# Potato256/my-mitsuba

Measured on AMD Instinct MI355X. Metric: Msamples/sec at 1280x720x256spp, 1/2/4/8 MI355X; per-pixel L1 vs CPU ref, higher is better.
Workload: dtype f32; 1 GPU; C3 bunny x15, 1,041,765 triangles, roughconductor Cu GGX 0.2, 15 instances flattened to world-space triangles; resolution=1280x720, spp=256, max_depth=8, parallelism=film tiles round-robin over 1 GPU(s), kd_build=host, kd_refs=4723933, kd_stop_prims=4

## Files before the change

include/mtsg.h:

```cpp
#ifndef MTSG_H
#define MTSG_H

#include <stdint.h>
#include <stddef.h>

#ifdef __cplusplus
extern "C" {
#endif

#define MTSG_ABI_VERSION 8

enum {
    MTSG_OK             = 0,
    MTSG_ERR_INVALID    = -1,
    MTSG_ERR_DEVICE     = -2,
    MTSG_ERR_OOM        = -3,
    MTSG_ERR_CANCELLED  = -4,
    MTSG_ERR_NODEVICE   = -5,
    MTSG_ERR_TRAVERSAL  = -6
};


typedef struct mtsg_kdnode {
    uint32_t combined;
// ... 333 lines not shown

int  mtsg_render_device(mtsg_scene *scene, const mtsg_render_params *params,
                        float *rgbaw_device);

int  mtsg_tile_windows(mtsg_scene *scene, const mtsg_render_params *params,
                       uint32_t *ntiles, int32_t *window);
int  mtsg_render_device_tiles(mtsg_scene *scene, const mtsg_render_params *params,
                              float *windows_device);

int  mtsg_set_tile_list(mtsg_scene *scene, const int32_t *keys, uint32_t n);

int  mtsg_device_alloc(mtsg_scene *scene, size_t bytes, void **out);
int  mtsg_device_free(mtsg_scene *scene, void *ptr);
int  mtsg_device_memset(mtsg_scene *scene, void *ptr, size_t bytes);
int  mtsg_device_to_host(mtsg_scene *scene, void *dst, const void *src, size_t bytes);

void mtsg_cancel(mtsg_scene *scene);

void mtsg_cancel_clear(mtsg_scene *scene);

typedef void (*mtsg_tile_fn)(void *user, int32_t key, int32_t x, int32_t y, int32_t w, int32_t h);
int  mtsg_set_tile_callback(mtsg_scene *scene, mtsg_tile_fn fn, void *user);

int  mtsg_set_flags(mtsg_scene *scene, uint32_t flags);
int  mtsg_get_stats(mtsg_scene *scene, mtsg_stats *out);
int  mtsg_debug_wavetimes(mtsg_scene *scene, uint64_t *out, uint32_t max_launches, uint32_t *waves);
int  mtsg_debug_stragglers(mtsg_scene *scene, float *out, uint32_t max_rays);

int  mtsg_set_batch_paths(mtsg_scene *scene, uint32_t paths);

#define MTSG_DEFAULT_FINISH_PATHS 524288u
int  mtsg_set_finish_paths(mtsg_scene *scene, uint32_t paths);

enum {
    MTSG_OPT_TRACE_REFILL = 1,
    MTSG_OPT_FINISH_SHADE_MIN = 2,
    MTSG_OPT_LANES = 3,
    MTSG_OPT_STAGGER = 4,
    MTSG_OPT_SHADE_GENERIC = 5,
    MTSG_OPT_RAY_ORDER = 6,
    MTSG_OPT_CAMERA_DIFFS = 7
};
int  mtsg_set_option(mtsg_scene *scene, int32_t key, int64_t value);

enum { MTSG_EMITTER_SET_AREA = 0, MTSG_EMITTER_SET_ENVMAP = 1, MTSG_EMITTER_SET_ALL = 2 };
int  mtsg_scene_kernel_sets(mtsg_scene *scene, int32_t *material_set, int32_t *emitter_set);

typedef struct mtsg_test_knobs {
    int32_t stack_cap, restart_guard, restart_limit, limit_shadow_only;
    int32_t no_instance_prefilter;
} mtsg_test_knobs;
int  mtsg_set_test_knobs(mtsg_scene *scene, const mtsg_test_knobs *knobs);

int  mtsg_env_eval(mtsg_scene *scene, uint32_t n, const float *dirs, const float *rx, const float *ry, float *out);

int  mtsg_tex_eval(mtsg_scene *scene, int tex, uint32_t n, const float *uv, const float *duv, float *out);

int  mtsg_om_query(mtsg_scene *scene, uint32_t n, const float *dirs, const float *o1, const float *o2, int32_t *ids,
                   int32_t *vis);

typedef struct mtsg_kd_build_params {
    float traversal_cost;
    float query_cost;
    float empty_space_bonus;
    int32_t stop_prims;
    int32_t max_depth;
    int32_t pad;
} mtsg_kd_build_params;

typedef struct mtsg_kd_tree {
    mtsg_kdnode *nodes;
    uint32_t n_nodes;
    uint32_t *indices;
    uint32_t n_indices;
// ... 88 lines not shown
```

my-mitsuba_amd/csrc/kernels.h:

```cpp
#pragma once
#include <hip/hip_runtime.h>

#include <stdint.h>

#include "../../include/mtsg.h"
#include "device_math.h"
#include "envmap.h"
#include "sampler.h"

namespace mtsg {

struct DevCamera;
struct DevScene {
    const uint4 *__restrict__ blocks;
    uint2 root2;
    const float4 *__restrict__ triL;
    const float4 *__restrict__ vpos;
    const float4 *__restrict__ vnrm;
    const uint4 *__restrict__ tidx;
    const float4 *__restrict__ shrec;
    const mtsg_rect *__restrict__ rects;
    const float4 *__restrict__ rectM;
    const float4 *__restrict__ rectSh;
    const float4 *__restrict__ emitRect;
    const mtsg_shape *__restrict__ shapes;
    const mtsg_bsdf *__restrict__ bsdfs;
    const mtsg_emitter *__restrict__ emitters;
    const float *__restrict__ emitter_cdf;
    const float *__restrict__ emitter_tri_cdf;
    uint32_t n_emitters, n_tri, n_bsdfs;
    float bmin[3], bmax[3];
    int has_env;
    DevEnv env;
    const uint32_t *qmcPrimes, *qmcOff;
    const uint16_t *qmcPerm;
    const float4 *__restrict__ inst;
    const mtsg_texture *__restrict__ textures;
    const float *__restrict__ tex_texels;
    const float4 *__restrict__ ttex;
    int cam_diffs;
    int cam_env_diffs;
    const DevCamera *__restrict__ camDev;
    float camO[3], camNear, camFar;
    int camCompact;
    uint4 *__restrict__ instSave;
    const mtsg_om *__restrict__ om;
    const uint32_t *__restrict__ om_bits;
    uint32_t capFlat, capGrp, capTop, rstGuard, rstMax, rstMaxC;
    uint32_t instPrefilter;
    uint32_t instKeyStride;
};

struct DevCamera {
    float s2c[16];
    float c2w[12];
// ... 64 lines not shown
    hipStream_t stream;
    const DevScene *S;
    const DevIntegrator *I;
    const DevBatch *B;
    const DevPaths *P;
    int bounce, qin;
    uint32_t nIdentity;
    int hasAlpha;
    uint32_t shadeMin;
    bool env, ext, inst;
    int mats;
    bool emx = false;
};
template <int SMP> void launch_shade_smp(const ShadeLaunch &a);
template <int SMP> void launch_finish_smp(const ShadeLaunch &a);
#define MTSG_DECLARE_LAUNCHERS(SMP) \
    template <> void launch_shade_smp<SMP>(const ShadeLaunch &a); \
    template <> void launch_finish_smp<SMP>(const ShadeLaunch &a);
MTSG_DECLARE_LAUNCHERS(MTSG_SAMPLER_INDEPENDENT)
MTSG_DECLARE_LAUNCHERS(MTSG_SAMPLER_HALTON)
MTSG_DECLARE_LAUNCHERS(MTSG_SAMPLER_HAMMERSLEY)
MTSG_DECLARE_LAUNCHERS(MTSG_SAMPLER_LDSAMPLER)
MTSG_DECLARE_LAUNCHERS(MTSG_SAMPLER_SOBOL)
int finish_blocks_per_cu(bool mats);
struct FlatTraceLaunch {
    dim3 grid, tieGrid;
    hipStream_t stream;
    const DevScene *S;
    const DevPaths *P;
    int cIn, sIn;
    uint32_t n;
    unsigned long long *wt;
    bool count, knobs, refill32, tie;
};
void launch_trace_flat(const FlatTraceLaunch &a);
int trace_flat_blocks_per_cu();

struct DevAov {
    int m;
    int pathChild;
    int nf;
    int kind[MTSG_MAX_SUBINTEGRATORS];
    int child[MTSG_MAX_SUBINTEGRATORS];
    float undef[MTSG_MAX_SUBINTEGRATORS][3];
    float w2c[16];
    const mtsg_aov_bsdf *bsdfs;
    const mtsg_aov_shape *shapes;
    const uint32_t *elems;
    float *planes;
    size_t cap;
};
struct FieldsLaunch {
    hipStream_t stream;
    const DevScene *S;
    const DevCamera *C;
    const DevIntegrator *I;
    const DevBatch *B;
    const DevPaths *P;
    const DevAov *A;
    float *film;
    int blockW, blockH, win;
};
void launch_fields(const FieldsLaunch &a);
void launch_splat_multi(const FieldsLaunch &a);

struct DevDirect {
// ... 387 lines not shown
    __syncthreads();
#endif
#if MTSG_LDS_PAD
    if (threadIdx.x == 0) ((volatile uint32_t *)s_ldsPad)[(S.n_tri & 0xFFFFu) % (MTSG_LDS_PAD / 4)] = 0u;
#endif
}
DEV uint32_t lane_here() {
    uint32_t l;
    asm volatile("v_mbcnt_lo_u32_b32 %0, -1, 0\n\tv_mbcnt_hi_u32_b32 %0, -1, %0" : "=v"(l));
    return l;
}
DEV uint32_t rank_below(unsigned long long m) {
    return __builtin_amdgcn_mbcnt_hi((uint32_t)(m >> 32), __builtin_amdgcn_mbcnt_lo((uint32_t)m, 0u));
}
struct SpecStack {
    DEV static uint32_t at(uint32_t k) { return k * TRACE_BLOCK + lane_here(); }
    DEV void push(uint32_t k, uint2 node, float t) const {
        const uint32_t i = at(k);
        s_specNode[i] = node;
        s_specT[i] = t;
    }
    DEV uint2 node(uint32_t k) const { return s_specNode[at(k)]; }
    DEV float t(uint32_t k) const { return s_specT[at(k)]; }
};

DEV float4 miss_record() {
    float4 m;
    uint32_t inf = 0x7F800000u, z = 0u, ff = 0xFFFFFFFFu;
    asm volatile("" : "+v"(inf), "+v"(z), "+v"(ff));
    m.x = __uint_as_float(inf); m.y = __uint_as_float(z); m.z = __uint_as_float(z); m.w = __uint_as_float(ff);
    return m;
}

DEV bool spec_init(const DevScene &S, float3 o, float3 d, float rayMint, float rayMaxt, bool shadow, SpecRay &r) {
    r.o = o;
    r.d = d;
    r.inv = mk3(rcp_exact(d.x), rcp_exact(d.y), rcp_exact(d.z));
    const uint32_t dneg = (d.x <= 0.0f ? 1u : 0u) | (d.y <= 0.0f ? 2u : 0u) | (d.z <= 0.0f ? 4u : 0u);
    float nearT = -INFINITY, farT = INFINITY;
    bool ok = true;
#pragma unroll
    for (int i = 0; i < 3; ++i) {
        const float oi = comp(o, i), di = comp(d, i), ii = comp(r.inv, i);
        const bool par = di == 0.0f;
        const float t1 = (S.bmin[i] - oi) * ii, t2 = (S.bmax[i] - oi) * ii;
        nearT = par ? nearT : fmaxf(fminf(t1, t2), nearT);
        farT = par ? farT : fminf(fmaxf(t1, t2), farT);
        ok &= !par | ((oi >= S.bmin[i]) & (oi <= S.bmax[i]));
    }
    if (!ok || !(nearT <= farT)) return false;
    float m = fmaxf(fmaxf(fabsf(o.x), fabsf(o.y)), fabsf(o.z));
    if (!shadow) m = fmaxf(m, kEpsilon);
    const float rayMinT = rayMint == kEpsilon ? rayMint * m : rayMint;
    r.mint = fmaxf(nearT, rayMinT);
    r.best = fminf(farT, rayMaxt);
    if (!(r.best > r.mint)) return false;
    r.tmin = r.mint;
    r.tmax = r.best;
    r.cur = S.root2;
    r.rroot = S.root2;
    r.lfE = r.lfEnd = 0;
    r.lfTmax = -1.0f;
    r.bits = dneg << SB_DNEG | (shadow ? SB_SHADOW : 0u);
    r.mb = 0;
    r.bestKey = 0xFFFFFFFFu;
    return true;
}

DEV void spec_plan(const SpecRay &r, uint2 n, float &tsplit, bool &goLeft, bool &push) {
    const uint32_t axis = n.x & 3u;
    const float split = __uint_as_float(n.y);
    const bool a0 = axis == 0u, a1 = axis == 1u;
    const float ox = r.o.x, oy = r.o.y, oz = r.o.z, ix = r.inv.x, iy = r.inv.y, iz = r.inv.z;
    const float oa = a0 ? ox : (a1 ? oy : oz);
    const float ia = a0 ? ix : (a1 ? iy : iz);
    tsplit = (split - oa) * ia;
    if (tsplit != tsplit) tsplit = INFINITY;
    const bool belowFirst = (oa < split) | ((oa == split) & (bool)((r.bits >> (SB_DNEG + axis)) & 1u));
    const bool onlyFirst = (tsplit > r.tmax) | (tsplit <= 0.0f);
    const bool goSecond = !onlyFirst & (tsplit < r.tmin);
    push = !onlyFirst & !goSecond;
    goLeft = belowFirst != goSecond;
}

#ifndef MTSG_PUSHDOWN
#define MTSG_PUSHDOWN 0
#endif
DEV uint2 spec_take(SpecRay &r, const uint4 &pr, float tsplit, bool goLeft, bool push, SpecStack stk, uint32_t cap) {
    const uint2 c = goLeft ? make_uint2(pr.x, pr.y) : make_uint2(pr.z, pr.w);
#if MTSG_PUSHDOWN
    if (!push && !(r.bits & (SB_N | SB_DROPPED))) r.rroot = c;
#endif
    if (push) {
        const uint2 other = goLeft ? make_uint2(pr.z, pr.w) : make_uint2(pr.x, pr.y);
        const uint32_t b = r.bits, top = b & SB_TOP;
        stk.push(top, other, r.tmax);
        const bool full = (b & SB_N) == cap * SB_N1;
        r.bits = ((b & ~SB_TOP) | (top == cap - 1 ? 0u : top + 1u)) + (full ? SB_DROPPED - (b & SB_DROPPED) : SB_N1);
// ... 1 lines not shown
    }
    return c;
}

#ifndef MTSG_RECT_PEND
#define MTSG_RECT_PEND 0
#endif
#ifndef MTSG_RECT_PEND_I
#define MTSG_RECT_PEND_I 0
#endif
#ifndef MTSG_ENTER_BATCH
#define MTSG_ENTER_BATCH 8
#endif
#ifndef MTSG_POPSEL
#define MTSG_POPSEL 0
#endif
#ifndef MTSG_INST_MIN_IDLE
#define MTSG_INST_MIN_IDLE 16
#endif
#ifndef MTSG_EXIT_BATCH
#define MTSG_EXIT_BATCH 0
#endif
#ifndef MTSG_MAILBOX
#define MTSG_MAILBOX 1
#endif
#ifndef MTSG_TIE_INLINE
#define MTSG_TIE_INLINE 0
#endif
constexpr bool TIE_INLINE = MTSG_TIE_INLINE;
#ifndef MTSG_RETIRE_BATCH
#define MTSG_RETIRE_BATCH 1
#endif
constexpr bool RETIRE_BATCH = MTSG_RETIRE_BATCH;
__shared__ uint32_t s_mbPrev[TRACE_BLOCK];
DEV bool mailbox_tie(SpecRay &r, uint32_t mb, uint32_t sl, uint32_t id, const float4 *hitOut) {
    if (!(r.bits & SB_FOUND)) return true;
    const uint32_t bs = (mb >> 20) & 7u, ps = (mb >> 17) & 7u;
    const uint32_t bestId = ((const uint32_t *)hitOut)[3];
    if (id == bestId) {
        r.mb = (mb & ~(1u << bs)) | (0x100u << bs);
        return false;
    }
    if ((mb & 0x10000u) && id == s_mbPrev[lane_here()] && !(mb & (0x100u << ps))) {
        r.mb = mb;
        return false;
    }
    s_mbPrev[lane_here()] = bestId;
    r.mb = sl << 20 | bs << 17 | 0x10000u | ((mb & 0xFFu) | (1u << sl)) << 8;
    return true;
}
DEV bool mailbox_step(SpecRay &r, uint32_t key, bool isRect, uint32_t prim, bool h, float t, const float4 *hitOut) {
    const uint32_t mb = r.mb, tag = (key & 7u) << 20 | 0x101u << (key & 7u);
    r.mb = h ? (tag & 0x700000u) : ((tag & 0xFFFFu) | mb);
    if (h & (t == r.best)) h = mailbox_tie(r, mb, tag >> 20, isRect ? (0x80000000u | prim) : prim, hitOut);
    return h;
}

template <bool COUNT, bool MB = false>
DEV bool spec_iter(const DevScene &S, SpecRay &r, SpecStack stk, TraceCounts &cnt, float4 *hitOut, const TravLimits &L) {
    const uint2 n = r.cur;
    const bool inner = !(r.bits & SB_TRAVDONE) && !(n.x & 0x80000000u);
    const bool prim = r.lfE < r.lfEnd;
    const bool rootKind = inner && !(n.x & 4u);
    float tsplit;
    bool goLeft, push;
    spec_plan(r, n, tsplit, goLeft, push);
    const uint32_t base = inner ? (n.x >> 3) << ((~n.x >> 1) & 2u) : 0u;
    const uint32_t off = rootKind ? 2u - (uint32_t)goLeft : 0u;
    const uint32_t pi = prim ? r.lfE : 0u;
#if MTSG_LDS_TOP
    uint4 p0, pc;
    if (base < 20u) p0 = s_top[base]; else p0 = S.blocks[base];
    if (base + off < 20u) pc = s_top[base + off]; else pc = S.blocks[base + off];
#else
    const uint4 p0 = S.blocks[base], pc = S.blocks[base + off];
#endif
#if MTSG_RECT_PEND
    const bool rp = (r.bits & SB_RPEND) != 0;
    const float4 *rec = rp ? S.rectM + (size_t)(3u * r.rpend) : S.triL + (size_t)(3u * pi);
#else
    const float4 *rec = S.triL + (size_t)(3u * pi);
#endif
    const float4 f0 = rec[0], f1 = rec[1], f2 = rec[2];
    asm volatile("" ::"v"(p0.x), "v"(p0.y), "v"(p0.z), "v"(p0.w), "v"(pc.x), "v"(pc.y), "v"(pc.z), "v"(pc.w),
                 "v"(f0.x), "v"(f0.y), "v"(f0.z), "v"(f0.w),
                 "v"(f1.x), "v"(f1.y), "v"(f1.z), "v"(f1.w), "v"(f2.x), "v"(f2.y), "v"(f2.z), "v"(f2.w));
#if MTSG_RECT_PEND
    if (prim && !rp && __float_as_uint(f0.x) == MTSG_TRIACCEL_SHAPE) {
        r.rpend = __float_as_uint(f2.w);
        r.bits |= SB_RPEND;
    } else if (prim) {
        if (COUNT) { cnt.refs++; cnt.tests++; }
        float t, u, v;
        const bool isRect = rp;
        bool h;
        uint32_t key, pid;
        if (rp) {
            h = rect_test_rows(f0, f1, f2, r.o, r.d, r.mint, r.best, t, u, v);
            key = S.n_tri + r.rpend;
            pid = r.rpend;
            r.bits &= ~SB_RPEND;
        } else {
            h = tri_test(f0, f1, f2, r.o, r.d, r.mint, r.best, u, v, t);
            key = __float_as_uint(f2.z);
            pid = __float_as_uint(f2.w);
        }
#else
    if (prim) {
        if (COUNT) { cnt.refs++; cnt.tests++; }
        float t, u, v;
        bool h = tri_test(f0, f1, f2, r.o, r.d, r.mint, r.best, u, v, t);
        const bool isRect = __float_as_uint(f0.x) == MTSG_TRIACCEL_SHAPE;
        if (isRect) h = rect_test(S.rects[__float_as_uint(f2.w)], r.o, r.d, r.mint, r.best, t, u, v);
        const uint32_t key = __float_as_uint(f2.z), pid = __float_as_uint(f2.w);
#endif
#if MTSG_MAILBOX
        if (MB) h = mailbox_step(r, key, isRect, pid, h, t, hitOut);
        else r.bits |= (h & (t == r.best) & (key != r.bestKey)) ? SB_TIE : 0u;
        if (h) r.bestKey = key;
#endif
        if (h) {
            r.bits |= SB_FOUND;
            if (r.bits & SB_SHADOW) return true;
            r.best = t;
            stS(hitOut, make_float4(t, u, v, __uint_as_float(isRect ? (0x80000000u | pid) : pid)));
        }
        ++r.lfE;
    }
    if (inner) {
        if (COUNT) cnt.nodes++;
        const uint2 c = spec_take(r, p0, tsplit, goLeft, push, stk, L.capFlat);
        r.cur = c;
        if (rootKind && !(c.x & 0x80000000u)) {
            if (COUNT) cnt.nodes++;
            float ts2;
            bool gl2, push2;
            spec_plan(r, c, ts2, gl2, push2);
            r.cur = spec_take(r, pc, ts2, gl2, push2, stk, L.capFlat);
        }
    }
    const bool found = (r.bits & SB_FOUND) != 0;
    const bool leafDone = (r.lfTmax >= 0.0f) & (r.lfE >= r.lfEnd);
    if (leafDone & found & (r.best < r.lfTmax)) return true;
    r.lfTmax = leafDone ? -1.0f : r.lfTmax;
    const uint2 c = r.cur;
// ... 586 lines not shown
            if (__lane_id() == 63u) waveSum[tid >> 6] = incl;
        }
        __syncthreads();
        if (tid < (uint32_t)SORT_BINS) {
            uint32_t before = 0u;
            for (uint32_t w = 0; w < (tid >> 6); ++w) before += waveSum[w];
            hist[tid] = before + incl - v;
        }
        __syncthreads();
#pragma unroll
        for (int j = 0; j < PER; ++j) {
            const uint32_t pos = w0 + (uint32_t)j * SORT_BLOCK + tid;
            if (pos < n) P.orderBuf[w0 + hist[key[j]] + rank[j]] = pos;
        }
        __syncthreads();
    }
}

#ifndef MTSG_SHUFFLE
#define MTSG_SHUFFLE 0
#endif
DEV uint32_t shuffle_index(uint32_t x, uint32_t n) {
    if (n < 2) return x;
    const uint32_t m = 32u - __clz(n - 1u), mask = m >= 32 ? 0xFFFFFFFFu : (1u << m) - 1u;
    do {
        x = (x * 0x9E3779B1u + 0x7F4A7C15u) & mask;
        x ^= x >> ((m + 1) / 2);
        x = (x * 0x85EBCA6Bu) & mask;
        x ^= x >> ((m + 2) / 3);
    } while (x >= n);
    return x;
}

template <bool COUNT, int MIN_IDLE, bool INST, bool KNOBS>
DEV void trace_s_body(const DevScene &S, const DevPaths &P, int cIn, int sIn, uint32_t nIdentity, unsigned long long *wt) {
    const SpecStack stk{};
    const TravLimits L = trav_limits<KNOBS>(S);
    lds_top_init(S);
    const unsigned long long tStart = wt ? wall_clock64() : 0ull;
    const uint32_t nC = cIn == -1 ? nIdentity : (cIn >= 0 ? __atomic_load_n(&P.cnt[cnt_q(cIn)], __ATOMIC_RELAXED) : 0u);
    const uint32_t nS = sIn >= 0 ? __atomic_load_n(&P.cnt[cnt_s(sIn)], __ATOMIC_RELAXED) : 0u;
    Fetch F{&P.cnt[CNT_FETCH], nC + nS, blockIdx.x % XGROUPS, 0, max(1u, gridDim.x / XGROUPS * GUIDE_SPLIT), FETCH};
    TraceCounts cc{0, 0, 0, 0, 0, 0, 0, 0, 0}, cs{0, 0, 0, 0, 0, 0, 0, 0, 0};
    uint32_t poolBase = 0, poolLeft = 0;
    bool exhausted = false;
    bool active = false;
    uint32_t idx = 0;
    uint32_t inst = 0;
    TopSave ts;
    uint32_t iters = 0;
    uint32_t n0 = 0, t0c = 0, r0 = 0;
    unsigned long long tExh = 0;
    uint32_t drainIters = 0;
    SpecRay r;
    bool pend = false;
    auto retire = [&]() {
        if (MTSG_MAILBOX && !(!INST && TIE_INLINE) && (r.bits & (SB_TIE | SB_SHADOW | SB_MBRUN)) == SB_TIE) {
            if (COUNT) atomicAdd(&P.ctr[CTR_TIE_RETRACES], 1ull);
            P.tie[atomicAdd(&P.cnt[CNT_TIE], 1u)] = idx;
        }
        if (COUNT) {
            const bool sh = (r.bits & SB_SHADOW) != 0;
            if (!INST) {
                const uint32_t nr = (r.bits >> SB_RST_SHIFT) & SB_RST_MASK;
                if (nr) atomicAdd(&P.ctr[CTR_RESTARTS + sh], (unsigned long long)nr);
                if (nr > L.rstGuard) {
                    atomicAdd(&P.ctr[CTR_GUARD_RAYS + sh], 1ull);
                    atomicAdd(&P.ctr[CTR_GUARD_STEPS + sh], (unsigned long long)(nr - L.rstGuard));
                }
            }
// ... 18 lines not shown
        }
    };
    for (;;) {
        unsigned long long idle = __ballot(!active);
        if ((uint32_t)__popcll(idle) < (uint32_t)MIN_IDLE && __any(active)) idle = 0;
        if (RETIRE_BATCH && idle && pend) {
            retire();
            pend = false;
        }
        while (idle && !exhausted) {
            if (poolLeft == 0 && !F.next(FETCH, poolBase, poolLeft)) {
                exhausted = true;
                if (WT_DRAIN && wt) tExh = wall_clock64();
                break;
            }
            const uint32_t nIdle = (uint32_t)__popcll(idle);
            const uint32_t take = min(nIdle, poolLeft);
            const uint32_t rank = rank_below(idle);
            if (!active && rank < take) {
                const uint32_t i = poolBase + rank;
                const bool shadow = i >= nC;
                idx = shadow ? i - nC : (P.order ? P.order[i] : i);
#if MTSG_SHUFFLE
                if (!shadow || MTSG_SHUFFLE == 2) idx = shuffle_index(idx, shadow ? nS : nC);
#endif
                float4 ro, rd;
                if (shadow) {
                    ro = ldS(P.sh_o + idx);
                    rd = ldS(P.sh_d + idx);
                    const float mint = rd.w; rd.w = ro.w; ro.w = mint;
                } else {
                    load_closest_ray(S, P, idx, !INST && P.camEnc != 0, ro, rd);
                }
                if (spec_init(S, xyz(ro), xyz(rd), ro.w, rd.w, shadow, r)) {
                    active = true;
                    if (COUNT) {
                        iters = 0;
                        const TraceCounts &k = shadow ? cs : cc;
                        n0 = k.nodes; t0c = k.tests; r0 = k.restarts;
                    }
                } else if (shadow) {
                    shadow_unoccluded(P, idx);
                } else if (!(rd.w < 0.0f)) {
                    stS(&P.hit[idx], miss_record());
                }
                if (INST && !shadow) P.hitInst[idx] = 0xFFFFFFFFu;
            }
            poolBase += take;
            poolLeft -= take;
            idle = __ballot(!active);
            if (take == nIdle) break;
        }
        if (!__any(active)) {
            if (exhausted) break;
            continue;
        }
        if (COUNT) {
            const uint2 n = r.cur;
            const bool inner = active && !(r.bits & SB_TRAVDONE) && !(n.x & 0x80000000u);
            const bool prim = active && r.lfE < r.lfEnd;
            const bool anyInner = __any(inner), anyPrim = __any(prim);
            const uint32_t nActive = (uint32_t)__popcll(__ballot(active));
            if (__lane_id() == 0) { cc.wsteps += 1; cc.wnodes += anyInner; cc.wtests += anyPrim; cc.wactive += nActive; }
        }
        if (WT_DRAIN && wt && exhausted) ++drainIters;
        bool done = false;
        if (active) {
            if (INST) {
                const bool sh = (r.bits & SB_SHADOW) != 0;
                if (COUNT && sh) done = spec_iter_i<COUNT>(S, r, cs, P, idx, L, inst, ts);
                else done = spec_iter_i<COUNT>(S, r, cc, P, idx, L, inst, ts);
            } else if (TIE_INLINE && (r.bits & SB_MBRUN)) {
                done = spec_iter<false, true>(S, r, stk, cc, P.hit + idx, L);
            } else {
                if (COUNT && (r.bits & SB_SHADOW)) done = spec_iter<COUNT>(S, r, stk, cs, P.hit + idx, L);
                else done = spec_iter<COUNT>(S, r, stk, cc, P.hit + idx, L);
            }
        }
        if (COUNT && active) ++iters;
        if (done && MTSG_MAILBOX && !INST && TIE_INLINE && (r.bits & (SB_TIE | SB_SHADOW | SB_MBRUN)) == SB_TIE) {
            if (COUNT) atomicAdd(&P.ctr[CTR_TIE_RETRACES], 1ull);
            float4 ro, rd;
            load_closest_ray(S, P, idx, P.camEnc != 0, ro, rd);
            spec_init(S, xyz(ro), xyz(rd), ro.w, rd.w, false, r);
            r.bits |= SB_MBRUN;
            done = false;
        }
        if (done) {
            active = false;
            if (RETIRE_BATCH) pend = true;
            else retire();
        }
    }
    flush_counts<COUNT>(P.ctr, cc);
    flush_counts<COUNT>(P.ctr + CTR_SHADOW, cs);
    if (COUNT && INST) {
        unsigned long long vi[2] = {cc.inst, cs.inst};
        for (int k = 0; k < 2; ++k) {
            for (int o2 = 32; o2 > 0; o2 >>= 1) vi[k] += __shfl_down(vi[k], o2);
            if (lane_id() == 0) atomicAdd(P.ctr + CTR_INST_VISITS + k, vi[k]);
        }
    }
    if (wt && __lane_id() == 0) {
        wt[WT_WORDS * blockIdx.x] = tStart;
        wt[WT_WORDS * blockIdx.x + 1] = wall_clock64();
        wt[WT_WORDS * blockIdx.x + 2] = tExh;
        wt[WT_WORDS * blockIdx.x + 3] = drainIters;
    }
}

#ifndef MTSG_FLAT_REGS
#define MTSG_FLAT_REGS 0
#endif
#ifndef MTSG_FLAT_SGPRS
#define MTSG_FLAT_SGPRS 98
#endif
#define FLAT_TRACE_ATTR __launch_bounds__(TRACE_BLOCK) __attribute__((amdgpu_num_vgpr(64), amdgpu_num_sgpr(MTSG_FLAT_SGPRS)))
template <bool COUNT, int MIN_IDLE, bool INST = false, bool KNOBS = false>
__global__ void __launch_bounds__(TRACE_BLOCK)
__attribute__((amdgpu_waves_per_eu(INST ? (COUNT ? 1 : MTSG_INST_WAVES) : (MTSG_FLAT_REGS && !COUNT ? 0 : MTSG_SPEC_WAVES))))
k_trace_s(DevScene S, DevPaths P, int cIn, int sIn, uint32_t nIdentity, unsigned long long *wt) {
    trace_s_body<COUNT, MIN_IDLE, INST, KNOBS>(S, P, cIn, sIn, nIdentity, wt);
}

#ifndef MTSG_TILE_MORTON
#define MTSG_TILE_MORTON 1
#endif
__host__ __device__ inline void tile_pix(uint32_t pix, int &lx, int &ly) {
#if MTSG_TILE_MORTON
    lx = (int)((pix & 1u) | ((pix >> 1) & 2u) | ((pix >> 2) & 4u) | ((pix >> 3) & 8u));
    ly = (int)(((pix >> 1) & 1u) | ((pix >> 2) & 2u) | ((pix >> 3) & 4u) | ((pix >> 4) & 8u));
#else
    lx = (int)(pix % TILE);
    ly = (int)(pix / TILE);
#endif
}
DEV void slot_pixel(const DevBatch &B, uint32_t slot, int &x, int &y, uint32_t &s) {
    const uint32_t pix = slot & (TILE * TILE - 1);
    const uint32_t rest = slot >> 8;
    const uint32_t sl = rest % B.ns;
    const uint32_t tl = rest / B.ns;
    int tx, ty;
    tile_of_key(batch_key(B, B.tile0 + (int)tl), B.tiles_x, tx, ty, B.skew);
    int lx, ly;
    tile_pix(pix, lx, ly);
    x = B.rect_x + tx * TILE + lx;
    y = B.rect_y + ty * TILE + ly;
    s = B.s0 + sl;
}

DEV float3 camera_near(const DevCamera &C, int x, int y, float a, float b) {
    const float sx = ((float)x + a) * C.inv_res_x, sy = ((float)y + b) * C.inv_res_y;
    const float *m = C.s2c;
    float px = m[0] * sx + m[1] * sy + m[3], py = m[4] * sx + m[5] * sy + m[7];
    float pz = m[8] * sx + m[9] * sy + m[11], pw = m[12] * sx + m[13] * sy + m[15];
// ... 1979 lines not shown
```

my-mitsuba_amd/csrc/mtsg.hip:

```cpp
#include <hip/hip_runtime.h>

#include <algorithm>
#include <atomic>
#include <cstdio>
#include <cstdlib>
#include <cstring>
#include <mutex>
#include <string>
#include <unordered_map>
#include <vector>
#include <chrono>
#include <functional>

#include "../../include/mtsg.h"
#include "device_math.h"
#include "envmap.h"
#include "sampler.h"

#include "kernels.h"
#include "render_plan.h"

static_assert(PLAN_TILE == TILE, "render_plan.h plans in tiles of kernels.h's edge");

namespace {
// ... 39 lines not shown
struct mtsg_scene {
    int device = 0;
    mtsg_tile_fn tileFn = nullptr;
    void *tileUser = nullptr;
    hipStream_t stream = nullptr;
    DevScene ds{};
    DevCamera cam{};
    std::vector<void *> allocs;
    uint32_t capacity = 0;
    uint32_t requestedBatch = 0;
    int lanes = MTSG_LANES;
    int stagger = 0;
    int lanesAlloc = 0;
    hipStream_t lstream[MTSG_MAX_LANES] = {};
    std::vector<int32_t> tileKeys;
    int32_t *tileKeysDev = nullptr;
    size_t tileKeysCap = 0;
    DevPaths LP[MTSG_MAX_LANES]{};
    std::vector<void *> batchAllocs;
    uint32_t *hostCnt = nullptr;
    int cuCount = 0;
    int traceGrid = 0, shadeGrid = 0, traceGridInst = 0, finishGrid = 0, finishGridMats = 0;
    uint32_t finishPaths = 0;
    uint32_t finishShadeMin = 16;
    uint32_t flags = 0;
    int samplerType = MTSG_SAMPLER_INDEPENDENT, samplerDim = 4;
    int qmcInv[2][3] = {{0, 0, 0}, {0, 0, 0}};
    int traceMode = 0;
    bool texDiffs = false, hasEnvmap = false, storeCamDiffs = false;
    int rayOrder = 0;
    float *dumpL = nullptr;
    std::atomic<int> cancel{0};
    bool knobs = false;
    mtsg_stats stats{};
    std::vector<hipEvent_t> evPool;
    size_t evUsed = 0;
    std::vector<std::pair<int, size_t>> timed;
    std::vector<unsigned long long> stragglers;
    unsigned long long *waveTimes = nullptr;
    uint32_t wtLaunches = 0;
    bool extBsdfs = false;
    int mats = MATS_ALL;
    bool shadeGeneric = false;
    int emitterSet = EM_AREA;
    uint32_t nTextures = 0;
    const uint32_t *sobolM = nullptr;
    const uint64_t *sobolVdc = nullptr, *sobolVdcInv = nullptr;
    uint64_t sobolScramble = 0;
    bool aovOn = false;
    DevAov aov{};
    std::vector<void *> aovAllocs;
    float *fieldPlanes = nullptr;
    size_t fieldCap = 0;
    int fieldCount = 0;
    uint32_t nShapes = 0;
    std::vector<int32_t> bsdfTexture;
    float *dumpMulti = nullptr;
    bool directOn = false;
    mtsg_direct_desc direct{};
    DevDirect fan{};
    std::vector<void *> fanAllocs;
    size_t fanClosest = 0, fanShadow = 0;
};

namespace {

// ... 90 lines not shown
    std::swap(P.aux, P.n_aux);
    std::swap(P.Lp, P.n_Lp);
    std::swap(P.meta, P.n_meta);
}

hipEvent_t next_event(mtsg_scene *s) {
    if (s->evUsed == s->evPool.size()) {
        hipEvent_t e;
        hipEventCreate(&e);
        s->evPool.push_back(e);
    }
    return s->evPool[s->evUsed++];
}

template <class F>
void timed_launch(mtsg_scene *s, int kind, hipStream_t st, F f) {
    if (!(s->flags & MTSG_FLAG_TIMING)) { f(); return; }
    size_t i0 = s->evUsed;
    hipEventRecord(next_event(s), st);
    f();
    hipEventRecord(next_event(s), st);
    s->timed.emplace_back(kind, i0);
}

template <bool COUNT>
void launch_trace_c(mtsg_scene *s, const DevPaths &P, int cIn, int sIn, uint32_t n, hipStream_t st) {
    dim3 g(s->traceGrid), blk(TRACE_BLOCK);
    unsigned long long *wt = nullptr;
    if ((s->flags & MTSG_FLAG_WAVETIME) && s->waveTimes && s->wtLaunches < WT_MAX_LAUNCHES && !s->ds.inst)
        wt = s->waveTimes + (size_t)WT_WORDS * s->traceGrid * s->wtLaunches++;
    const dim3 tg(std::max<unsigned>(1u, (unsigned)s->traceGrid / 4u));
    if (!s->ds.inst) {
        FlatTraceLaunch a{g, tg, st, &s->ds, &P, cIn, sIn, n, wt, COUNT, s->knobs, s->traceMode == 1,
                          MTSG_MAILBOX && cIn != -2 && !TIE_INLINE};
        launch_trace_flat(a);
        return;
    }
    if (s->knobs && !COUNT)
        hipLaunchKernelGGL((k_trace_s<false, MTSG_INST_MIN_IDLE, true, true>), dim3(s->traceGridInst), blk, 0, st, s->ds, P, cIn, sIn, n, wt);
    else hipLaunchKernelGGL((k_trace_s<COUNT, MTSG_INST_MIN_IDLE, true>), dim3(s->traceGridInst), blk, 0, st, s->ds, P, cIn, sIn, n, wt);
    if (MTSG_MAILBOX && cIn != -2) hipLaunchKernelGGL(k_tie_i, tg, blk, 0, st, s->ds, P);
}
void launch_trace(mtsg_scene *s, bool count, const DevPaths &P, int cIn, int sIn, uint32_t n, hipStream_t st) {
    if (count) launch_trace_c<true>(s, P, cIn, sIn, n, st);
    else launch_trace_c<false>(s, P, cIn, sIn, n, st);
}

ShadeLaunch shade_args(mtsg_scene *s, const DevIntegrator &I, const DevBatch &B, const DevPaths &P, int b, int qin, hipStream_t st,
                       dim3 grid, dim3 block) {
    ShadeLaunch a;
    a.grid = grid;
    a.block = block;
    a.stream = st;
    a.S = &s->ds;
    a.I = &I;
    a.B = &B;
    a.P = &P;
    a.bounce = b;
    a.qin = qin;
    a.nIdentity = B.nslots;
    a.hasAlpha = s->cam.has_alpha || s->aovOn;
    a.shadeMin = s->finishShadeMin;
    a.env = (s->ds.has_env & 1) != 0;
    a.ext = s->extBsdfs;
    a.inst = s->ds.inst != nullptr;
    a.emx = s->emitterSet == EM_ALL;
    a.mats = (s->shadeGeneric || a.emx) ? (int)MATS_ALL : s->mats;
// ... 1086 lines not shown
            return fail(rc);
        ds.textures = dtex; ds.tex_texels = dtt;
        s->nTextures = d->n_textures;
        s->extBsdfs = true;
    }
    if (d->tri_uv && d->tri_dpdv) {
        std::vector<float4> tt((size_t)3 * std::max(1u, d->n_triangles), make_float4(0, 0, 0, 0));
        for (uint32_t t = 0; t < d->n_triangles; ++t) {
            const float *uv = d->tri_uv + 6 * (size_t)t, *dv = d->tri_dpdv + 3 * (size_t)t;
            tt[3 * t] = make_float4(uv[0], uv[1], uv[2], uv[3]);
            tt[3 * t + 1] = make_float4(uv[4], uv[5], dv[0], dv[1]);
            tt[3 * t + 2] = make_float4(dv[2], 0.f, 0.f, 0.f);
        }
        float4 *dttex;
        if ((rc = up(tt.data(), tt.size(), &dttex))) return fail(rc);
        ds.ttex = dttex;
    }
    s->nShapes = d->n_shapes;
    s->bsdfTexture.resize(d->n_bsdfs);
    for (uint32_t i = 0; i < d->n_bsdfs; ++i) s->bsdfTexture[i] = d->bsdfs[i].texture;
    s->texDiffs = texDiffs;
    s->hasEnvmap = d->has_envmap != 0;
    ds.om = nullptr; ds.om_bits = nullptr;
    if (d->om) {
        if (!d->om_bits) { g_err = "occupancy maps without their bits"; return fail(MTSG_ERR_INVALID); }
        mtsg_om *dom; uint32_t *dbits;
        if ((rc = up(d->om, 1, &dom)) ||
            (rc = up(d->om_bits, (size_t)MTSG_OM_COUNT * MTSG_OM_SIZE * MTSG_OM_SIZE * (MTSG_OM_SIZE / 32), &dbits)))
            return fail(rc);
        ds.om = dom; ds.om_bits = dbits;
    }
    ds.n_emitters = d->n_emitters;
    ds.n_tri = d->n_triangles;
    ds.n_bsdfs = d->n_bsdfs;
    for (int k = 0; k < 3; ++k) { ds.bmin[k] = d->aabb_min[k]; ds.bmax[k] = d->aabb_max[k]; }
    DevCamera &c = s->cam;
    const mtsg_camera &hc = d->camera;
    memcpy(c.s2c, hc.sample_to_camera, sizeof(c.s2c));
    memcpy(c.c2w, hc.camera_to_world, sizeof(c.c2w));
    c.near_clip = hc.near_clip; c.far_clip = hc.far_clip; c.inv_res_x = hc.inv_res_x; c.inv_res_y = hc.inv_res_y;
    c.film_w = hc.film_w; c.film_h = hc.film_h;
    c.filter_radius = hc.filter_radius; c.filter_scale = hc.filter_scale; c.border = hc.border;
    c.has_alpha = hc.has_alpha;
    memcpy(c.filter_values, hc.filter_values, sizeof(c.filter_values));
    memcpy(c.dx, hc.dx, sizeof(c.dx));
    memcpy(c.dy, hc.dy, sizeof(c.dy));
    c.crop_w = hc.crop_w; c.crop_h = hc.crop_h;
    c.lens = hc.sensor_type == MTSG_SENSOR_THINLENS ? 1 : 0;
    c.aperture_radius = hc.aperture_radius; c.focus_distance = hc.focus_distance;
    ds.camO[0] = c.c2w[3]; ds.camO[1] = c.c2w[7]; ds.camO[2] = c.c2w[11];
    ds.camNear = c.near_clip; ds.camFar = c.far_clip;
    ds.camCompact = (ds.inst || c.lens) ? 0 : 1;
    c.compact = ds.camCompact;
    camera_diff_mode(s);
    {
        DevCamera *dc;
        if ((rc = up(&s->cam, 1, &dc))) return fail(rc);
        ds.camDev = dc;
    }
    s->samplerType = d->sampler.type;
    s->samplerDim = d->sampler.dimension;
    if (s->samplerType < MTSG_SAMPLER_INDEPENDENT || s->samplerType > MTSG_SAMPLER_SOBOL) {
        g_err = "unknown sampler type";
        return fail(MTSG_ERR_INVALID);
    }
    if (s->samplerType == MTSG_SAMPLER_HALTON || s->samplerType == MTSG_SAMPLER_HAMMERSLEY) {
// ... 111 lines not shown
    return MTSG_OK;
}

int mtsg_set_option(mtsg_scene *s, int32_t key, int64_t value) {
    if (!s) { g_err = "null scene"; return MTSG_ERR_INVALID; }
    switch (key) {
        case MTSG_OPT_TRACE_REFILL:
            if (value != 16 && value != 32) { g_err = "MTSG_OPT_TRACE_REFILL: 16 or 32 idle lanes"; return MTSG_ERR_INVALID; }
            s->traceMode = value == 32 ? 1 : 0;
            return MTSG_OK;
        case MTSG_OPT_FINISH_SHADE_MIN:
            if (value < 1 || value > 64) { g_err = "MTSG_OPT_FINISH_SHADE_MIN: 1..64 lanes"; return MTSG_ERR_INVALID; }
            s->finishShadeMin = (uint32_t)value;
            return MTSG_OK;
        case MTSG_OPT_LANES:
            if (value < 1 || value > MTSG_MAX_LANES) { g_err = "MTSG_OPT_LANES: 1..4 concurrent batches"; return MTSG_ERR_INVALID; }
            s->lanes = (int)value;
            return MTSG_OK;
        case MTSG_OPT_STAGGER:
            if (value < 0 || value > 16) { g_err = "MTSG_OPT_STAGGER: 0..16 bounces"; return MTSG_ERR_INVALID; }
            s->stagger = (int)value;
            return MTSG_OK;
        case MTSG_OPT_SHADE_GENERIC:
            s->shadeGeneric = value != 0;
            return MTSG_OK;
        case MTSG_OPT_RAY_ORDER:
            if (value < 0 || value > 1) { g_err = "MTSG_OPT_RAY_ORDER: 0 (append order) or 1 (direction-sorted windows)"; return MTSG_ERR_INVALID; }
            s->rayOrder = (int)value;
            return MTSG_OK;
        case MTSG_OPT_CAMERA_DIFFS:
            if (value < 0 || value > 1) { g_err = "MTSG_OPT_CAMERA_DIFFS: 0 (recomputed on a miss) or 1 (stored)"; return MTSG_ERR_INVALID; }
            s->storeCamDiffs = value != 0;
            camera_diff_mode(s);
            return MTSG_OK;
        default:
            g_err = "unknown option key " + std::to_string(key);
            return MTSG_ERR_INVALID;
    }
}

int mtsg_set_flags(mtsg_scene *s, uint32_t flags) {
    if (!s) return MTSG_ERR_INVALID;
    s->flags = flags;
    return MTSG_OK;
}

int mtsg_get_stats(mtsg_scene *s, mtsg_stats *out) {
    if (!s || !out) return MTSG_ERR_INVALID;
    *out = s->stats;
    return MTSG_OK;
}

int mtsg_debug_wavetimes(mtsg_scene *s, uint64_t *out, uint32_t max_launches, uint32_t *waves) {
    if (!s || !waves || (!out && max_launches)) return MTSG_ERR_INVALID;
    *waves = (uint32_t)s->traceGrid;
    const uint32_t n = std::min(max_launches, s->wtLaunches);
    if (n && s->waveTimes &&
        hipMemcpy(out, s->waveTimes, (size_t)WT_WORDS * s->traceGrid * n * sizeof(uint64_t), hipMemcpyDeviceToHost) != hipSuccess)
        return MTSG_ERR_DEVICE;
    return (int)s->wtLaunches;
}

int mtsg_debug_stragglers(mtsg_scene *s, float *out, uint32_t max_rays) {
    if (!s || (!out && max_rays)) return MTSG_ERR_INVALID;
    const uint32_t n = (uint32_t)(s->stragglers.size() / 8);
    for (uint32_t k = 0; k < std::min(n, max_rays); ++k) {
// ... 554 lines not shown
```

my-mitsuba_amd/csrc/trace_flat.hip:

```cpp
#pragma clang diagnostic ignored "-Wunused-function"
#include "kernels.h"

#if MTSG_FLAT_REGS
namespace {
#define FLAT_TRACE_KERNEL(MIN_IDLE, KNOBS)                                                                               \
    template <>                                                                                                          \
    __global__ void FLAT_TRACE_ATTR k_trace_s<false, MIN_IDLE, false, KNOBS>(DevScene S, DevPaths P, int cIn, int sIn,   \
                                                                             uint32_t nIdentity, unsigned long long *wt) { \
        trace_s_body<false, MIN_IDLE, false, KNOBS>(S, P, cIn, sIn, nIdentity, wt);                                      \
    }
FLAT_TRACE_KERNEL(16, false)
FLAT_TRACE_KERNEL(32, false)
FLAT_TRACE_KERNEL(16, true)
#undef FLAT_TRACE_KERNEL
}
#endif

namespace mtsg {

template <bool COUNT>
static void launch_flat(const FlatTraceLaunch &a) {
    const dim3 blk(TRACE_BLOCK);
    if (a.knobs && !COUNT) hipLaunchKernelGGL((k_trace_s<false, 16, false, true>), a.grid, blk, 0, a.stream, *a.S, *a.P, a.cIn, a.sIn, a.n, a.wt);
    else if (a.refill32) hipLaunchKernelGGL((k_trace_s<COUNT, 32>), a.grid, blk, 0, a.stream, *a.S, *a.P, a.cIn, a.sIn, a.n, a.wt);
    else hipLaunchKernelGGL((k_trace_s<COUNT, 16>), a.grid, blk, 0, a.stream, *a.S, *a.P, a.cIn, a.sIn, a.n, a.wt);
    if (a.tie) {
        if (a.knobs) hipLaunchKernelGGL((k_tie<true>), a.tieGrid, blk, 0, a.stream, *a.S, *a.P);
        else hipLaunchKernelGGL((k_tie<false>), a.tieGrid, blk, 0, a.stream, *a.S, *a.P);
    }
}

void launch_trace_flat(const FlatTraceLaunch &a) {
    if (a.count) launch_flat<true>(a);
    else launch_flat<false>(a);
}

int trace_flat_blocks_per_cu() {
    int perCU = 0;
    if (hipOccupancyMaxActiveBlocksPerMultiprocessor(&perCU, (const void *)k_trace_s<false, 16>, TRACE_BLOCK, 0) != hipSuccess) return 0;
    return perCU;
}

}
```

my-mitsuba_amd/mtsg.py:

```python
from __future__ import annotations

import ctypes as C
import os

import numpy as np

PKG_DIR = os.path.dirname(os.path.abspath(__file__))
REPO_DIR = os.path.dirname(PKG_DIR)

MTSG_OK = 0
MTSH_INSTANCING_FLATTEN = 0
MTSH_INSTANCING_TWO_LEVEL = 1
MTSG_FLAG_TIMING = 1
MTSG_FLAG_COUNT = 2
MTSG_FLAG_WAVETIME = 4
MTSG_OPT_TRACE_REFILL = 1
MTSG_OPT_FINISH_SHADE_MIN = 2
MTSG_OPT_LANES = 3
MTSG_OPT_STAGGER = 4
MTSG_OPT_SHADE_GENERIC = 5
MTSG_OPT_RAY_ORDER = 6
MTSG_OPT_CAMERA_DIFFS = 7
MTSG_INTEGRATOR_PATH = 0
MTSG_INTEGRATOR_PATH2_OM = 1
MTSG_INTEGRATOR_DIRECT = 2
MTSG_INTEGRATOR_AO = 3
MTSG_EMITTER_AREA, MTSG_EMITTER_ENVMAP, MTSG_EMITTER_POINT, MTSG_EMITTER_SPOT = 1, 2, 3, 4
MTSG_EMITTER_DIRECTIONAL, MTSG_EMITTER_CONSTANT = 5, 6


class RenderParams(C.Structure):
    _fields_ = [
        ("max_depth", C.c_int32), ("rr_depth", C.c_int32),
        ("strict_normals", C.c_int32), ("hide_emitters", C.c_int32),
        ("spp", C.c_uint32), ("seed", C.c_uint32),
        ("tile_x", C.c_int32), ("tile_y", C.c_int32),
        ("tile_w", C.c_int32), ("tile_h", C.c_int32),
        ("tile_stride", C.c_int32), ("tile_offset", C.c_int32),
        ("integrator", C.c_int32), ("om_strategy", C.c_int32), ("om_mis", C.c_int32), ("om_jitter", C.c_int32),
    ]

    def copy(self) -> "RenderParams":
        p = RenderParams()
        C.memmove(C.byref(p), C.byref(self), C.sizeof(RenderParams))
        return p


class TestKnobs(C.Structure):
    _fields_ = [("stack_cap", C.c_int32), ("restart_guard", C.c_int32), ("restart_limit", C.c_int32),
                ("limit_shadow_only", C.c_int32), ("no_instance_prefilter", C.c_int32)]


class Stats(C.Structure):
    _fields_ = [
        ("ms_total", C.c_double), ("ms_trace_closest", C.c_double),
# ... 1058 lines not shown
```

Before: 1671 Msamples/s.

## Test scene rectangles once at ray setup instead of in kd-tree leaves

When the scene has at most two analytic rectangles, they are intersected against each ray in spec_init before traversal starts. This tightens the ray's max t early, and shadow rays that hit a rectangle end without traversing. The leaf loop then drops its per-primitive rectangle branch. A separate leaf-rect kernel is kept for scenes that do not qualify, at the cost of an extra kernel instantiation and a fixed per-ray rectangle test.

```diff
diff --git a/include/mtsg.h b/include/mtsg.h
--- a/include/mtsg.h
+++ b/include/mtsg.h
@@ -389,6 +389,7 @@
 #define MTSG_DEFAULT_FINISH_PATHS 524288u
 int  mtsg_set_finish_paths(mtsg_scene *scene, uint32_t paths);
 
+#define MTSG_RECT_SETUP_CAP 2u
 enum {
     MTSG_OPT_TRACE_REFILL = 1,
     MTSG_OPT_FINISH_SHADE_MIN = 2,
@@ -396,7 +397,8 @@
     MTSG_OPT_STAGGER = 4,
     MTSG_OPT_SHADE_GENERIC = 5,
     MTSG_OPT_RAY_ORDER = 6,
-    MTSG_OPT_CAMERA_DIFFS = 7
+    MTSG_OPT_CAMERA_DIFFS = 7,
+    MTSG_OPT_RECT_SETUP = 8
 };
 int  mtsg_set_option(mtsg_scene *scene, int32_t key, int64_t value);
 
diff --git a/my-mitsuba_amd/csrc/kernels.h b/my-mitsuba_amd/csrc/kernels.h
--- a/my-mitsuba_amd/csrc/kernels.h
+++ b/my-mitsuba_amd/csrc/kernels.h
@@ -21,6 +21,7 @@
     const float4 *__restrict__ shrec;
     const mtsg_rect *__restrict__ rects;
     const float4 *__restrict__ rectM;
+    uint32_t n_rect;
     const float4 *__restrict__ rectSh;
     const float4 *__restrict__ emitRect;
     const mtsg_shape *__restrict__ shapes;
@@ -151,6 +152,7 @@
     uint32_t n;
     unsigned long long *wt;
     bool count, knobs, refill32, tie;
+    bool rectSetup;
 };
 void launch_trace_flat(const FlatTraceLaunch &a);
 int trace_flat_blocks_per_cu();
@@ -604,7 +606,10 @@
     return m;
 }
 
-DEV bool spec_init(const DevScene &S, float3 o, float3 d, float rayMint, float rayMaxt, bool shadow, SpecRay &r) {
+template <bool RS = false>
+DEV bool spec_init(const DevScene &S, float3 o, float3 d, float rayMint, float rayMaxt, bool shadow, SpecRay &r,
+                   float4 *hitOut = nullptr) {
+    if (RS) r.bits = 0u;
     r.o = o;
     r.d = d;
     r.inv = mk3(rcp_exact(d.x), rcp_exact(d.y), rcp_exact(d.z));
@@ -636,6 +641,30 @@
     r.bits = dneg << SB_DNEG | (shadow ? SB_SHADOW : 0u);
     r.mb = 0;
     r.bestKey = 0xFFFFFFFFu;
+    if (RS) {
+        float4 rec = make_float4(0.0f, 0.0f, 0.0f, 0.0f);
+        bool found = false;
+        const uint32_t nR = S.n_rect;
+        for (uint32_t k = 0; k < nR; ++k) {
+            const float4 *m = S.rectM + 3u * k;
+            float t, u, v;
+            const bool h = rect_test_rows(m[0], m[1], m[2], r.o, r.d, r.mint, r.best, t, u, v);
+            const uint32_t key = S.n_tri + k;
+            r.bits |= (h & (t == r.best) & (key != r.bestKey)) ? SB_TIE : 0u;
+            r.bestKey = h ? key : r.bestKey;
+            r.best = (h & !shadow) ? t : r.best;
+            rec = h ? make_float4(t, u, v, __uint_as_float(0x80000000u | k)) : rec;
+            found |= h;
+        }
+        if (found) {
+            if (shadow) {
+                r.bits = SB_FOUND;
+                return false;
+            }
+            r.bits |= SB_FOUND;
+            stS(hitOut, rec);
+        }
+    }
     return true;
 }
 
@@ -703,6 +732,11 @@
 #define MTSG_RETIRE_BATCH 1
 #endif
 constexpr bool RETIRE_BATCH = MTSG_RETIRE_BATCH;
+#ifndef MTSG_RECT_SETUP
+#define MTSG_RECT_SETUP 1
+#endif
+constexpr bool RECT_SETUP = MTSG_RECT_SETUP && !MTSG_RECT_PEND && !MTSG_TIE_INLINE;
+constexpr uint32_t RECT_SETUP_CAP = MTSG_RECT_SETUP_CAP;
 __shared__ uint32_t s_mbPrev[TRACE_BLOCK];
 DEV bool mailbox_tie(SpecRay &r, uint32_t mb, uint32_t sl, uint32_t id, const float4 *hitOut) {
     if (!(r.bits & SB_FOUND)) return true;
@@ -727,8 +761,9 @@
     return h;
 }
 
-template <bool COUNT, bool MB = false>
+template <bool COUNT, bool MB = false, bool RS = false>
 DEV bool spec_iter(const DevScene &S, SpecRay &r, SpecStack stk, TraceCounts &cnt, float4 *hitOut, const TravLimits &L) {
+    static_assert(!(RS && (MB || MTSG_RECT_PEND)), "the mailbox retrace and MTSG_RECT_PEND test rectangles in the leaves");
     const uint2 n = r.cur;
     const bool inner = !(r.bits & SB_TRAVDONE) && !(n.x & 0x80000000u);
     const bool prim = r.lfE < r.lfEnd;
@@ -778,10 +813,10 @@
         }
 #else
     if (prim) {
-        if (COUNT) { cnt.refs++; cnt.tests++; }
+        if (COUNT) { cnt.refs++; cnt.tests += !(RS && __float_as_uint(f0.x) == MTSG_TRIACCEL_SHAPE); }
         float t, u, v;
         bool h = tri_test(f0, f1, f2, r.o, r.d, r.mint, r.best, u, v, t);
-        const bool isRect = __float_as_uint(f0.x) == MTSG_TRIACCEL_SHAPE;
+        const bool isRect = !RS && __float_as_uint(f0.x) == MTSG_TRIACCEL_SHAPE;
         if (isRect) h = rect_test(S.rects[__float_as_uint(f2.w)], r.o, r.d, r.mint, r.best, t, u, v);
         const uint32_t key = __float_as_uint(f2.z), pid = __float_as_uint(f2.w);
 #endif
@@ -1434,10 +1469,11 @@
     return x;
 }
 
-template <bool COUNT, int MIN_IDLE, bool INST, bool KNOBS>
+template <bool COUNT, int MIN_IDLE, bool INST, bool KNOBS, bool LEAF_RECTS = false>
 DEV void trace_s_body(const DevScene &S, const DevPaths &P, int cIn, int sIn, uint32_t nIdentity, unsigned long long *wt) {
     const SpecStack stk{};
     const TravLimits L = trav_limits<KNOBS>(S);
+    constexpr bool RS = RECT_SETUP && !INST && !KNOBS && !LEAF_RECTS;
     lds_top_init(S);
     const unsigned long long tStart = wt ? wall_clock64() : 0ull;
     const uint32_t nC = cIn == -1 ? nIdentity : (cIn >= 0 ? __atomic_load_n(&P.cnt[cnt_q(cIn)], __ATOMIC_RELAXED) : 0u);
@@ -1522,13 +1558,14 @@
                 } else {
                     load_closest_ray(S, P, idx, !INST && P.camEnc != 0, ro, rd);
                 }
-                if (spec_init(S, xyz(ro), xyz(rd), ro.w, rd.w, shadow, r)) {
+                if (spec_init<RS>(S, xyz(ro), xyz(rd), ro.w, rd.w, shadow, r, P.hit + idx)) {
                     active = true;
                     if (COUNT) {
                         iters = 0;
                         const TraceCounts &k = shadow ? cs : cc;
                         n0 = k.nodes; t0c = k.tests; r0 = k.restarts;
                     }
+                } else if (RS && (r.bits & SB_FOUND)) {
                 } else if (shadow) {
                     shadow_unoccluded(P, idx);
                 } else if (!(rd.w < 0.0f)) {
@@ -1563,8 +1600,8 @@
             } else if (TIE_INLINE && (r.bits & SB_MBRUN)) {
                 done = spec_iter<false, true>(S, r, stk, cc, P.hit + idx, L);
             } else {
-                if (COUNT && (r.bits & SB_SHADOW)) done = spec_iter<COUNT>(S, r, stk, cs, P.hit + idx, L);
-                else done = spec_iter<COUNT>(S, r, stk, cc, P.hit + idx, L);
+                if (COUNT && (r.bits & SB_SHADOW)) done = spec_iter<COUNT, false, RS>(S, r, stk, cs, P.hit + idx, L);
+                else done = spec_iter<COUNT, false, RS>(S, r, stk, cc, P.hit + idx, L);
             }
         }
         if (COUNT && active) ++iters;
@@ -1611,6 +1648,11 @@
 __attribute__((amdgpu_waves_per_eu(INST ? (COUNT ? 1 : MTSG_INST_WAVES) : (MTSG_FLAT_REGS && !COUNT ? 0 : MTSG_SPEC_WAVES))))
 k_trace_s(DevScene S, DevPaths P, int cIn, int sIn, uint32_t nIdentity, unsigned long long *wt) {
     trace_s_body<COUNT, MIN_IDLE, INST, KNOBS>(S, P, cIn, sIn, nIdentity, wt);
+}
+template <bool COUNT, int MIN_IDLE>
+__global__ void __launch_bounds__(TRACE_BLOCK) __attribute__((amdgpu_waves_per_eu(MTSG_SPEC_WAVES)))
+k_trace_s_leaf(DevScene S, DevPaths P, int cIn, int sIn, uint32_t nIdentity, unsigned long long *wt) {
+    trace_s_body<COUNT, MIN_IDLE, false, false, true>(S, P, cIn, sIn, nIdentity, wt);
 }
 
 #ifndef MTSG_TILE_MORTON
diff --git a/my-mitsuba_amd/csrc/mtsg.hip b/my-mitsuba_amd/csrc/mtsg.hip
--- a/my-mitsuba_amd/csrc/mtsg.hip
+++ b/my-mitsuba_amd/csrc/mtsg.hip
@@ -95,6 +95,7 @@
     float *dumpL = nullptr;
     std::atomic<int> cancel{0};
     bool knobs = false;
+    bool rectSetupOpt = true, rectSetupOk = false;
     mtsg_stats stats{};
     std::vector<hipEvent_t> evPool;
     size_t evUsed = 0;
@@ -251,7 +252,7 @@
     const dim3 tg(std::max<unsigned>(1u, (unsigned)s->traceGrid / 4u));
     if (!s->ds.inst) {
         FlatTraceLaunch a{g, tg, st, &s->ds, &P, cIn, sIn, n, wt, COUNT, s->knobs, s->traceMode == 1,
-                          MTSG_MAILBOX && cIn != -2 && !TIE_INLINE};
+                          MTSG_MAILBOX && cIn != -2 && !TIE_INLINE, s->rectSetupOpt && s->rectSetupOk};
         launch_trace_flat(a);
         return;
     }
@@ -1404,6 +1405,13 @@
     }
     ds.n_emitters = d->n_emitters;
     ds.n_tri = d->n_triangles;
+    ds.n_rect = d->n_rects;
+    s->rectSetupOk = MTSG_RECT_SETUP && d->n_rects <= RECT_SETUP_CAP;
+    for (uint32_t r = 0; r < d->n_rects && s->rectSetupOk; ++r) {
+        const mtsg_triaccel &ta = d->triaccel[d->n_triangles + r];
+        s->rectSetupOk = ta.k == MTSG_TRIACCEL_SHAPE && ta.prim_index == r && ta.shape_index < d->n_shapes &&
+                         d->shapes[ta.shape_index].type == MTSG_SHAPE_RECT;
+    }
     ds.n_bsdfs = d->n_bsdfs;
     for (int k = 0; k < 3; ++k) { ds.bmin[k] = d->aabb_min[k]; ds.bmax[k] = d->aabb_max[k]; }
     DevCamera &c = s->cam;
@@ -1581,6 +1589,10 @@
             if (value < 0 || value > 1) { g_err = "MTSG_OPT_CAMERA_DIFFS: 0 (recomputed on a miss) or 1 (stored)"; return MTSG_ERR_INVALID; }
             s->storeCamDiffs = value != 0;
             camera_diff_mode(s);
+            return MTSG_OK;
+        case MTSG_OPT_RECT_SETUP:
+            if (value < 0 || value > 1) { g_err = "MTSG_OPT_RECT_SETUP: 0 (rectangles tested in the leaves) or 1 (at ray setup)"; return MTSG_ERR_INVALID; }
+            s->rectSetupOpt = value != 0;
             return MTSG_OK;
         default:
             g_err = "unknown option key " + std::to_string(key);
diff --git a/my-mitsuba_amd/csrc/trace_flat.hip b/my-mitsuba_amd/csrc/trace_flat.hip
--- a/my-mitsuba_amd/csrc/trace_flat.hip
+++ b/my-mitsuba_amd/csrc/trace_flat.hip
@@ -22,6 +22,8 @@
 static void launch_flat(const FlatTraceLaunch &a) {
     const dim3 blk(TRACE_BLOCK);
     if (a.knobs && !COUNT) hipLaunchKernelGGL((k_trace_s<false, 16, false, true>), a.grid, blk, 0, a.stream, *a.S, *a.P, a.cIn, a.sIn, a.n, a.wt);
+    else if (!a.rectSetup && a.refill32) hipLaunchKernelGGL((k_trace_s_leaf<COUNT, 32>), a.grid, blk, 0, a.stream, *a.S, *a.P, a.cIn, a.sIn, a.n, a.wt);
+    else if (!a.rectSetup) hipLaunchKernelGGL((k_trace_s_leaf<COUNT, 16>), a.grid, blk, 0, a.stream, *a.S, *a.P, a.cIn, a.sIn, a.n, a.wt);
     else if (a.refill32) hipLaunchKernelGGL((k_trace_s<COUNT, 32>), a.grid, blk, 0, a.stream, *a.S, *a.P, a.cIn, a.sIn, a.n, a.wt);
     else hipLaunchKernelGGL((k_trace_s<COUNT, 16>), a.grid, blk, 0, a.stream, *a.S, *a.P, a.cIn, a.sIn, a.n, a.wt);
     if (a.tie) {
diff --git a/my-mitsuba_amd/mtsg.py b/my-mitsuba_amd/mtsg.py
--- a/my-mitsuba_amd/mtsg.py
+++ b/my-mitsuba_amd/mtsg.py
@@ -21,6 +21,8 @@
 MTSG_OPT_SHADE_GENERIC = 5
 MTSG_OPT_RAY_ORDER = 6
 MTSG_OPT_CAMERA_DIFFS = 7
+MTSG_OPT_RECT_SETUP = 8
+MTSG_RECT_SETUP_CAP = 2
 MTSG_INTEGRATOR_PATH = 0
 MTSG_INTEGRATOR_PATH2_OM = 1
 MTSG_INTEGRATOR_DIRECT = 2
```

Measured after the change: 1785 Msamples/s, median of 6. +6.8%, better.
